# supyuxiang/Inference-Time-Scaling-for-Diffusion-Models-beyond-Scaling-Denoising-Steps

Measured on AMD Instinct MI355X. Metric: candidate-images/sec at T=1000, CIFAR-10 32x32 UNet, N=256, 1/2/4/8 MI355X, higher is better.
Workload: dtype bf16; 1 GPU; random-search round: N=256/GPU candidates x T=1000 DDPM steps, Arch A UNet 32x32 (ch128 [1,2,3,4] attn[2] nrb2), Oracle verifier; model=DDPM UNet (Diffusion/Model.py) Arch A, global_batch=256, seq_len=1000, parallelism=candidate-dp1, T=1000, graph=True, n_local=256

## Files before the change

### inference-time-scaling-for-diffusion-models-beyond-scaling-denoising-steps_amd/csrc/conv.hip

```cpp
#include <algorithm>
#include <type_traits>

#include "common.h"

namespace itsd {

constexpr int CONV_BM = 128;
constexpr int CONV_BN = 128;
constexpr int ROWB = 128;
constexpr int TILEB = 128 * ROWB;
constexpr int EROW = 132;
constexpr int EPI_BYTES = 128 * EROW * 4 + 8 * 2 * 128 * 4;
constexpr int SMEM_BYTES = (2 * 2 * TILEB > EPI_BYTES) ? 2 * 2 * TILEB : EPI_BYTES;
int g_fuse_gn = 1;
int g_conv_dbg = 0;
int g_conv_variant = 2;
int g_small_conv = 1;
int g_conv1x1 = 1;
int g_small_8x8 = 1;
int g_small_wide = 1;
int g_splitk = 1;
int g_gn_wide = 1;
int g_p4_w = 7;
int g_num_cus = 256;
// ... 1152 lines not shown
    wait_vmcnt<4>();
    __builtin_amdgcn_s_barrier();
    issue_w(s0 + 2);
    if constexpr (ST) {
      asm volatile("" ::: "memory");
      load_chunk(cc + 1);
      asm volatile("" ::: "memory");
    }
    mma_tap(s0, 0);
#pragma unroll 1
    for (int tap = 1; tap < 8; ++tap) {
      if (ST && tap <= 2) wait_vmcnt<4 + LPC>();
      else wait_vmcnt<4>();
      __builtin_amdgcn_s_barrier();
      issue_w(s0 + tap + 2);
      mma_tap(s0 + tap, tap);
    }
    wait_vmcnt<4>();
    __builtin_amdgcn_s_barrier();
    issue_w(s0 + 10);
    mma_tap(s0 + 8, 8);
    if constexpr (ST) {
      asm volatile("s_waitcnt lgkmcnt(0)" ::: "memory");
      __builtin_amdgcn_s_barrier();
      write_halo();
      asm volatile("s_waitcnt lgkmcnt(0)" ::: "memory");
    }
  };
  for (int cc = 0; cc + 1 < ncc; ++cc) run_chunk(cc, std::true_type{});
  run_chunk(ncc - 1, std::false_type{});
  wait_vmcnt<0>();
  __syncthreads();
  if (a.dbg & 16) return;
  conv_epilogue<T>(a, acc, smem, tileP, tileC);
}

#ifdef ITSD_STAMPS
__device__ unsigned long long g_stamps[1024 * 16 * 8];
__device__ __forceinline__ unsigned long long stamp() {
  __builtin_amdgcn_sched_barrier(0);
  const unsigned long long t = __builtin_amdgcn_s_memtime();
  __builtin_amdgcn_sched_barrier(0);
  return t;
}
#define STAMP(var) const unsigned long long var = stamp()
#define STAMP_ADD(slot, d) st[slot] += (d)
__device__ __forceinline__ void tl_stamp(int slot) {
  __builtin_amdgcn_sched_barrier(0);
  const unsigned long long t = (threadIdx.x >> 6) == 1 ? __builtin_amdgcn_s_memtime() : __builtin_amdgcn_s_memrealtime();
  if ((threadIdx.x & 63) == 0) g_stamps[((blockIdx.x & 1023) * 16 + (threadIdx.x >> 6)) * 8 + slot] = t;
  __builtin_amdgcn_sched_barrier(0);
}
#define TL(slot) tl_stamp(slot)
#else
#define TL(slot)
#define STAMP(var)
#define STAMP_ADD(slot, d)
#endif
constexpr int GNW_BN = 256;
constexpr int GNW_EPI = GNW_BN * EROW * 4 + (GNW_BN / 16) * 2 * CONV_BM * 4;
constexpr int GNW_SMEM = 160 * 1024;
static_assert(GNW_EPI <= GNW_SMEM, "epilogue tile");

constexpr float GN_L2E = -1.44269504f;
__device__ __forceinline__ float gn_silu_l2(float x, float a2, float b2) {
  const float t = __builtin_fmaf(x, a2, b2);
  return t * __builtin_amdgcn_rcpf(__builtin_fmaf(__builtin_amdgcn_exp2f(t), GN_L2E, GN_L2E));
}
__device__ __forceinline__ void gn_silu_x4(uint32_t xa, uint32_t xb, float a0, float a1, float a2, float a3,
                                           float b0, float b1, float b2, float b3, uint32_t zm, uint32_t& ya,
                                           uint32_t& yb) {
  float t0, t1, t2, t3, e0, e1, e2, e3;
  asm volatile(
      "v_lshlrev_b32 %2, 16, %10\n\t"
      "v_and_b32 %3, 0xffff0000, %10\n\t"
      "v_lshlrev_b32 %4, 16, %11\n\t"
      "v_and_b32 %5, 0xffff0000, %11\n\t"
      "v_fma_f32 %2, %2, %12, %16\n\t"
      "v_fma_f32 %3, %3, %13, %17\n\t"
      "v_fma_f32 %4, %4, %14, %18\n\t"
      "v_fma_f32 %5, %5, %15, %19\n\t"
      "v_exp_f32 %6, %2\n\t"
      "v_exp_f32 %7, %3\n\t"
      "v_exp_f32 %8, %4\n\t"
      "v_exp_f32 %9, %5\n\t"
      "v_fma_f32 %6, %6, %21, %21\n\t"
      "v_fma_f32 %7, %7, %21, %21\n\t"
      "v_fma_f32 %8, %8, %21, %21\n\t"
      "v_fma_f32 %9, %9, %21, %21\n\t"
      "v_rcp_f32 %6, %6\n\t"
      "v_rcp_f32 %7, %7\n\t"
      "v_rcp_f32 %8, %8\n\t"
      "v_rcp_f32 %9, %9\n\t"
      "v_mul_f32 %2, %2, %6\n\t"
      "v_mul_f32 %3, %3, %7\n\t"
      "v_mul_f32 %4, %4, %8\n\t"
      "v_mul_f32 %5, %5, %9\n\t"
      "v_cvt_pk_bf16_f32 %0, %2, %3\n\t"
      "v_cvt_pk_bf16_f32 %1, %4, %5\n\t"
      "v_and_b32 %0, %0, %20\n\t"
      "v_and_b32 %1, %1, %20"
      : "=&v"(ya), "=&v"(yb), "=&v"(t0), "=&v"(t1), "=&v"(t2), "=&v"(t3), "=&v"(e0), "=&v"(e1), "=&v"(e2),
        "=&v"(e3)
      : "v"(xa), "v"(xb), "v"(a0), "v"(a1), "v"(a2), "v"(a3), "v"(b0), "v"(b1), "v"(b2), "v"(b3), "v"(zm),
        "s"(GN_L2E));
}

template <int W> struct GnpCfg;
template <> struct GnpCfg<32> { static constexpr int NSEG = 1, ITEMS = 11, RES = 1; };
template <> struct GnpCfg<16> { static constexpr int NSEG = 1, ITEMS = 11, RES = 1; };
template <> struct GnpCfg<8> { static constexpr int NSEG = 4, ITEMS = 13, RES = 0; };


#ifndef ITSD_P4_M16
#define ITSD_P4_M16 2
#endif
#ifndef ITSD_P4_ZR8
#define ITSD_P4_ZR8 1
#endif
#ifndef ITSD_P5_SC_LAUNCH
#define ITSD_P5_SC_LAUNCH 7.5
#endif
#ifndef ITSD_P5_SWZ
#define ITSD_P5_SWZ 1
#endif
#ifndef ITSD_P4_SUBSWZ
#define ITSD_P4_SUBSWZ 1
#endif
#ifndef ITSD_P4_HSWZ
#define ITSD_P4_HSWZ 1
#endif
constexpr int P4_RING = 6;
constexpr int P4_BD = 2;
template <int W, int AB = 0>
__global__ __launch_bounds__(512, 1) void conv3x3_gn_p4_kernel(ConvArgs a) {
  typedef bf16_t T;
  constexpr bool SUB = (AB & 128) != 0, PLAIN = SUB || (AB & 2) != 0;
  constexpr bool SUB4 = SUB && (AB & 256) == 0;
  constexpr int NTAP = SUB4 ? 4 : 9, KST = 4 * NTAP;
  constexpr bool COMPACT = !SUB && (W == 8 || W == 16);
  constexpr int NSEG = GnpCfg<W>::NSEG, ITEMS = COMPACT ? 8 : GnpCfg<W>::ITEMS, RES = COMPACT ? 1 : GnpCfg<W>::RES;
  constexpr int W2 = W + 2;
  constexpr int THs = NSEG == 1 ? GNW_BN / W : W;
  constexpr int HS = (THs + 2) * W2;
  constexpr int HWs = THs * W;
  constexpr int TPS = 256 / NSEG, RPP = TPS / 8;
  constexpr int ZROW = GNW_BN;
  constexpr bool M16 = ITSD_P4_M16 >= 1 && RES && !SUB && (AB & 1) == 0 && (W == 32 || ITSD_P4_M16 >= 2);
  constexpr int ZROWS = COMPACT ? (M16 ? (ITSD_P4_ZR8 ? 72 : 65) : 1) : 0;
  auto hswz = [](int h) { return M16 && ITSD_P4_HSWZ ? (h & 6) : ((h >> 1) & 7); };
  constexpr bool CSWZ = ITSD_P4_SUBSWZ && !COMPACT && !M16 && W <= 16;
  constexpr int SC1 = 1, SC2 = W <= 8 ? 2 : 1;
  constexpr bool C96 = (AB & 512) != 0;
  constexpr int BM = C96 ? 96 : CONV_BM, HB = BM / 2, NCI = HB / 16;
  static_assert(!C96 || (M16 && COMPACT), "96-cout tiles: the 16x16x32 compact forms");
  constexpr int HALO = COMPACT ? (((GNW_BN + ZROWS) * ROWB + 1023) & ~1023) : NSEG * ITEMS * RPP * ROWB;
  constexpr int RESB = RES ? GNW_BN * CONV_BM * 2 : 0;
  static_assert(COMPACT ? ITEMS * RPP == HWs : ITEMS * RPP >= HS, "halo items cover the segment");
  constexpr int RING = ((AB & 64) || SUB) ? 4 : P4_RING, BD = (AB & 32) ? P4_BD + 1 : P4_BD;
  static_assert(KST % RING == 0, "ring slots repeat per chunk");
  __shared__ __attribute__((aligned(16))) char smem[2 * HALO + RESB + 2 * NSEG * CONV_BM * 4 + 4 * 64 * 4];
  char* const rlds = smem + 2 * HALO;
  float* const addv = (float*)(smem + 2 * HALO + RESB);
#ifdef ITSD_STAMPS
  {
    const unsigned hw = __builtin_amdgcn_s_getreg(4 | (4 << 6) | (1 << 11));
    if ((threadIdx.x & 63) == 0) g_stamps[((blockIdx.x & 1023) * 16 + 8 + (threadIdx.x >> 6)) * 8 + 1] = hw;
  }
#endif
  const int tid = threadIdx.x, lane = tid & 63;
  const int wid = __builtin_amdgcn_readfirstlane(tid >> 6);
  const int H = a.Hout;
  const int Cin = a.C1 + a.C2, ncc = Cin / 64, kpt = Cin >> 4;
  const int nTC = a.Cout / BM, nPT = a.M / GNW_BN, NT = (SUB ? 4 : 1) * nPT * nTC;
// ... 569 lines not shown
        float sm = 0.f;
#pragma unroll
        for (int i = 0; i < 2; ++i)
#pragma unroll
          for (int j = 0; j < 4; ++j)
#pragma unroll
            for (int r = 0; r < 16; ++r) sm += acc[i][j][r];
        if (sm == 1.2345f) ((float*)a.out)[0] = sm;
      }
      if constexpr (RES) {
        if (k + 1 < ntiles) init_acc(k + 1);
      } else {
#pragma unroll
        for (int i = 0; i < 2; ++i)
#pragma unroll
          for (int j = 0; j < 4; ++j)
#pragma unroll
            for (int r = 0; r < 16; ++r) acc[i][j][r] = 0.0f;
      }
      STAMP(e1);
      STAMP_ADD(6, e1 - e0);
    }
    if constexpr (RES) block_sync();
    P4_STAMP_OUT();
    return;
    }
  }

  const int tt = tid - 256, lch = tt & 7, sg = tt / TPS, lt = tt - sg * TPS;
  static_assert(COMPACT || NSEG * ITEMS * RPP > NSEG * HS, "a scratch row exists");
  if (a.dbg & (1 << 20)) __builtin_amdgcn_s_setprio(1);
  if (a.dbg & (1 << 21)) __builtin_amdgcn_s_setprio(2);
  const int dump = NSEG * HS * ROWB + (lch << 4);
  const int hrow0 = (COMPACT ? sg * HWs : sg * HS) + (lt >> 3), hrow1 = hrow0 + RPP;
  const int lds0 = hrow0 * ROWB + ((lch ^ hswz(hrow0)) << 4);
  const int lds1 = hrow1 * ROWB + ((lch ^ hswz(hrow1)) << 4);
  auto item_lds = [&](int j) {
    if constexpr (CSWZ) {
      const int r = (lt >> 3) + RPP * j, hy = r / W2, hx = r - hy * W2;
      return (sg * HS + r) * ROWB + ((lch ^ ((SC1 * hy + SC2 * hx) & 7)) << 4);
    }
    return ((j & 1) ? lds1 : lds0) + (j >> 1) * (2 * RPP * ROWB);
  };
  auto tile_y0img = [&](int k, int& img0, int& y0) {
    const int tileP = tile_p(k);
    img0 = tileP / (H * W);
    y0 = (tileP - img0 * H * W) / W;
  };
  int ipix[ITEMS];
  const float* cbase;
  int simg = 0;
  int gimg = -1;
  float* const gsw = (float*)(smem + 2 * HALO + RESB + 2 * NSEG * CONV_BM * 4) + (wid - 4) * 64;
  auto group_stats = [&](int img) __attribute__((always_inline)) {
    const int g = lane & 31, hf = Cin / 64, c0 = g * 2 * hf + (lane >> 5) * hf;
    const int HWi = H * W;
    const int sp1 = stat_spi(HWi, a.gn_spi1), sp2 = a.C2 ? stat_spi(HWi, a.gn_spi2) : 0;
    const int spm = sp1 > sp2 ? sp1 : sp2, np = hf >> 1, m = np * spm;
    double sm = 0.0, sq = 0.0;
    for (int b0 = 0; b0 < m; b0 += 8) {
      float2 vs[8], vq[8];
#pragma unroll
      for (int i = 0; i < 8; ++i) {
        const int it = b0 + i, q = it / np, cr = c0 + 2 * (it - q * np);
        const bool s1 = cr < a.C1;
        const bool ok = it < m && q < (s1 ? sp1 : sp2);
        const int c = ok ? cr : c0, qq = ok ? q : 0;
        const bool t1 = c < a.C1;
        const float* st = t1 ? a.gn_st1 : a.gn_st2;
        const int Cs = t1 ? a.C1 : a.C2, cs = t1 ? c : c - a.C1, sp = t1 ? sp1 : sp2;
        const long long slot = (long long)img * sp + qq;
        const float2 u0 = *(const float2*)(st + (slot * 2) * Cs + cs);
        const float2 u1 = *(const float2*)(st + (slot * 2 + 1) * Cs + cs);
        vs[i] = ok ? u0 : float2{0.f, 0.f};
        vq[i] = ok ? u1 : float2{0.f, 0.f};
      }
#pragma unroll
      for (int i = 0; i < 8; ++i) {
        sm += (double)vs[i].x + (double)vs[i].y;
        sq += (double)vq[i].x + (double)vq[i].y;
      }
    }
    sm += __shfl_xor(sm, 32, 64);
    sq += __shfl_xor(sq, 32, 64);
    const double E = (double)(Cin / 32) * HWi, mean = sm / E;
    double var = sq / E - mean * mean;
    var = var > 0.0 ? var : 0.0;
    if (lane < 32) {
      gsw[2 * g] = (float)mean;
      gsw[2 * g + 1] = (float)(1.0 / sqrt(var + 1e-5));
    }
  };
  auto geometry_pix = [&](int k) __attribute__((always_inline)) {
    int img0, y0;
    tile_y0img(k, img0, y0);
    int ltv = lt;
    asm volatile("" : "+v"(ltv));
#pragma unroll
    for (int j = 0; j < ITEMS; ++j) {
      const int r = (ltv >> 3) + RPP * j;
      if constexpr (COMPACT) {
        ipix[j] = (img0 + sg) * HWs + r;
      } else {
        const int hy = r / W2, hx = r - hy * W2, iy = y0 + hy - 1, ix = hx - 1;
        const bool ok = r < HS && iy >= 0 && iy < H && ix >= 0 && ix < W;
        ipix[j] = ok ? ((img0 + sg) * H + iy) * W + ix : 0;
      }
    }
    if constexpr (!PLAIN) cbase = a.gn_coef + ((size_t)(img0 + sg) * (Cin / 8) + lch) * 16;
    simg = img0 + sg;
  };
  static_assert(COMPACT || ITEMS * RPP - HS < RPP, "scratch rows only in the last item");
  const int waddr_last = (COMPACT || ((lt >> 3) + RPP * (ITEMS - 1)) < HS) ? item_lds(ITEMS - 1) : dump;
  auto waddr = [&](int j) { return j == ITEMS - 1 ? waddr_last : item_lds(j); };
  int inm = 0;
  auto geometry_emit = [&](int k) __attribute__((always_inline)) {
    int img0, y0;
    tile_y0img(k, img0, y0);
    int ltv = lt;
    asm volatile("" : "+v"(ltv));
    inm = 0;
    if constexpr (COMPACT) {
      inm = (1 << ITEMS) - 1;
      return;
    }
#pragma unroll
    for (int j = 0; j < ITEMS; ++j) {
      const int r = (ltv >> 3) + RPP * j;
      const int hy = r / W2, hx = r - hy * W2, iy = y0 + hy - 1, ix = hx - 1;
      const bool in = r >= HS || (iy >= 0 && iy < H && ix >= 0 && ix < W);
      inm |= (int)in << j;
    }
  };
  const int nrec1 = (int)std::min<long long>((long long)a.M * a.C1 * 2, 0x7fffffffLL);
  const int nrec2 = (int)std::min<long long>((long long)a.M * a.C2 * 2, 0x7fffffffLL);
  struct Src {
    __amdgpu_buffer_rsrc_t rs;
    uint32_t rowb, so;
  };
  auto src_of = [&](int cc, bool live) __attribute__((always_inline)) {
    const int ci0 = cc * 64;
    const bool s1 = ci0 < a.C1;
    Src c;
    c.rs = __builtin_amdgcn_make_buffer_rsrc(s1 ? (void*)a.src1 : (void*)a.src2, (short)0,
// ... 100 lines not shown
  };
  auto load_cn = [&](int ccx) __attribute__((always_inline)) {
    if constexpr (PLAIN) return;
    if (a.gn_fold) {
      const int c0 = ccx * 64 + 8 * lch;
      cn[0] = *(const f32x4*)(a.gn_gamma + c0);
      cn[1] = *(const f32x4*)(a.gn_gamma + c0 + 4);
      cn[2] = *(const f32x4*)(a.gn_beta + c0);
      cn[3] = *(const f32x4*)(a.gn_beta + c0 + 4);
    } else {
      const f32x4* cp = (const f32x4*)(cbase + ccx * 128);
#pragma unroll
      for (int q = 0; q < 4; ++q) cn[q] = cp[q];
    }
  };
  auto emit = [&](char* hbuf) __attribute__((always_inline)) {
    if (ccL == 0) geometry_emit(kL);
    bool opened = false;
    if (++ccL == ncc) {
      ccL = 0;
      if (++kL < ntiles) {
        geometry_pix(kL);
        opened = true;
      }
    }
    const bool live = kL < ntiles;
    load_cn(live ? ccL : 0);
    const Src nx = src_of(ccL, live);
    typedef __attribute__((ext_vector_type(2))) float f32x2;
    typedef __attribute__((ext_vector_type(2))) __bf16 bf16x2_t;
#pragma unroll
    for (int j = 0; j < ITEMS; ++j) {
      const uint32_t zm = (uint32_t)__builtin_amdgcn_sbfe(inm, j, 1);
      uint32_t yw[4];
      if constexpr (PLAIN) {
#pragma unroll
        for (int w = 0; w < 4; ++w) yw[w] = h[j][w] & zm;
      } else
#pragma unroll
      for (int hf = 0; hf < 2; ++hf)
        gn_silu_x4(h[j][2 * hf], h[j][2 * hf + 1], c[hf][0], c[hf][1], c[hf][2], c[hf][3], c[2 + hf][0],
                   c[2 + hf][1], c[2 + hf][2], c[2 + hf][3], zm, yw[2 * hf], yw[2 * hf + 1]);
      const u32x4 y = {yw[0], yw[1], yw[2], yw[3]};
      *(u32x4*)(hbuf + waddr(j)) = y;
      __builtin_amdgcn_sched_barrier(0);
      h[j] = __builtin_amdgcn_raw_buffer_load_b128(nx.rs, __umul24((uint32_t)ipix[j], nx.rowb) + lch * 16, nx.so, 0);
    }
    if (a.gn_fold && opened && simg != gimg) {
      group_stats(simg);
      gimg = simg;
    }
    prescale();
  };
  geometry_pix(0);
  {
    load_cn(0);
    const Src s0 = src_of(0, true);
#pragma unroll
    for (int j = 0; j < ITEMS; ++j)
      h[j] = __builtin_amdgcn_raw_buffer_load_b128(s0.rs, __umul24((uint32_t)ipix[j], s0.rowb) + lch * 16, s0.so, 0);
    if (a.gn_fold) group_stats(simg);
    gimg = simg;
    prescale();
  }
  if constexpr (COMPACT) {
    if (tt < 16) *(u32x4*)(smem + (tt >> 3) * HALO + ZROW * ROWB + ((tt & 7) << 4)) = u32x4{0u, 0u, 0u, 0u};
    if (M16 && ITSD_P4_ZR8) {
      const int r = (tt >> 3) & 15;
      *(u32x4*)(smem + (tt >> 7) * HALO + (ZROW + (r & 7) + (r >> 3) * 64) * ROWB + ((tt & 7) << 4)) = u32x4{0u, 0u, 0u, 0u};
    } else if (M16 && tt >= 16 && tt < 32) {
      *(u32x4*)(smem + ((tt >> 3) & 1) * HALO + (ZROW + 64) * ROWB + ((tt & 7) << 4)) = u32x4{0u, 0u, 0u, 0u};
    }
  }
  emit(smem);
#ifdef ITSD_STAMPS
  st[5] = stamp() - t_begin;
#endif
  block_sync();
  for (int q = 0, k = 0, cc = 0; q < nstages; ++q) {
    STAMP(h0);
    if (RES && cc == 1 && k > 0) {
      drain(k - 1);
      asm volatile("s_waitcnt lgkmcnt(0)" ::: "memory");
    }
    const bool res = RES && a.resid && cc == ncc - 1;
    if (res) res_dma(k);
    const int addv_cc = RES ? 0 : ncc - 1;
    if (cc == addv_cc && k + 1 < ntiles) stage_addv(k + 1, tt);
    if (q + 1 < nstages) emit(smem + ((q + 1) & 1) * HALO);
    if (res) {
      if (q + 1 < nstages) asm volatile("s_waitcnt vmcnt(%0)" ::"n"(ITEMS + 4) : "memory");
      else asm volatile("s_waitcnt vmcnt(0)" ::: "memory");
    }
#ifdef ITSD_STAMPS
    asm volatile("s_waitcnt lgkmcnt(0)" ::: "memory");
#endif
    STAMP(h1);
    STAMP_ADD(3, h1 - h0);
    block_sync();
    if (++cc == ncc) {
      cc = 0;
      ++k;
    }
  }
  if constexpr (RES) {
    block_sync();
    drain(ntiles - 1);
  }
  P4_STAMP_OUT();
}

template <int W> struct Gp5Cfg {
  static constexpr int HW = W * W;
  static constexpr bool ROWS = HW > 128;
// ... 60 lines not shown
  auto chunk_lo = [&](int z) { return z < S ? (nch * z) / S : (nchx * (z - S)) / S2; };
  auto chunk_hi = [&](int z) { return z < S ? (nch * (z + 1)) / S : (nchx * (z + 1 - S)) / S2; };
  auto block_sync = [&]() {
    asm volatile("s_waitcnt lgkmcnt(0)" ::: "memory");
    __builtin_amdgcn_s_barrier();
    asm volatile("" ::: "memory");
  };

  if (wid < 4) {
    const int rl = lane & 31, hh = lane >> 5;
    const int cw = CB == 128 ? wid : wid % CWB, jb0 = CB == 128 ? 0 : (wid / CWB) * NJW;
    int hb[NJW];
    int hq[NJW];
#pragma unroll
    for (int j = 0; j < NJW; ++j) {
      const int pl = (jb0 + j) * 32 + rl, seg = pl / SPX, rem = pl - seg * SPX, y = rem / W;
      hb[j] = seg * HS + y * W2 + (rem - y * W);
      hq[j] = SC1 * y + SC2 * (rem - y * W);
    }
    auto bunit = [&](int j, int h, int ky, int kx) {
      return W <= 16 && ITSD_P5_SWZ ? (hq[j] + SC1 * ky + SC2 * kx) & 7 : (h >> 1) & 7;
    };
    const uint32_t ablk = (uint32_t)(9 * kpt) * 1024;
    const __amdgpu_buffer_rsrc_t wrs = __builtin_amdgcn_make_buffer_rsrc((void*)a.wfrag, (short)0, 0x7fffffff, 0x00020000);
    const uint32_t avo = (uint32_t)lane * 16 + (uint32_t)cw * ablk;
    auto abase = [&](int tc, int cc) -> uint32_t { return (uint32_t)(tc * CWB) * ablk + (uint32_t)cc * 4 * 1024; };
    auto load_a = [&](uint32_t base, int st, u32x4& dst) __attribute__((always_inline)) {
#if defined(ITSD_DIAG) && defined(P5_AB)
      if constexpr ((P5_AB & 8) != 0) {
        dst = u32x4{(uint32_t)st, 0u, 0u, 0u};
        return;
      }
#endif
      dst = __builtin_amdgcn_raw_buffer_load_b128(wrs, avo, base + (uint32_t)((st >> 2) * kpt + (st & 3)) * 1024, 0);
    };
    f32x16 acc[NJW];
    u32x4 ra[P5_RING];
    const __amdgpu_buffer_rsrc_t wrx = __builtin_amdgcn_make_buffer_rsrc((void*)a.sc_wfrag, (short)0, 0x7fffffff, 0x00020000);
    const uint32_t ablkx = (uint32_t)(nchx * 4) * 1024;
    auto load_ax = [&](int tc, int cc, int st, u32x4& dst) __attribute__((always_inline)) {
      dst = __builtin_amdgcn_raw_buffer_load_b128(wrx, (uint32_t)lane * 16,
                                                  (uint32_t)(tc * CWB + cw) * ablkx + (uint32_t)(cc * 4 + st) * 1024, 0);
    };
    bool ring = false;
    {
      int tp, tc, z;
      item_of(0, tp, tc, z);
      if (z < S) {
        const uint32_t ab0 = abase(tc, chunk_lo(z));
#pragma unroll
        for (int s0 = 0; s0 < P5_RING - 1; ++s0) load_a(ab0, s0, ra[s0]);
        ring = true;
      }
    }
    block_sync();
    TL(1);
    int q = 0;
    for (int k = 0; k < nit; ++k) {
      int tp, tc, z;
      item_of(k, tp, tc, z);
      const int c0 = chunk_lo(z), c1 = chunk_hi(z);
#pragma unroll
      for (int j = 0; j < NJW; ++j)
#pragma unroll
        for (int r = 0; r < 16; ++r) acc[j][r] = 0.0f;
#if defined(ITSD_DIAG) && defined(P5_CHAINS2)
      f32x16 acc2[NJW];
#pragma unroll
      for (int j = 0; j < NJW; ++j)
#pragma unroll
        for (int r = 0; r < 16; ++r) acc2[j][r] = 0.0f;
#endif
      if (z >= S) {
#pragma unroll
        for (int st = 0; st < 4; ++st) load_ax(tc, c0, st, ra[st]);
        auto chunk1 = [&](auto pc, int cc) __attribute__((always_inline)) {
          constexpr int P = decltype(pc)::value;
          if (cc + 1 < c1) {
#pragma unroll
            for (int st = 0; st < 4; ++st) load_ax(tc, cc + 1, st, ra[4 * (1 - P) + st]);
          }
          int tx[NJW];
#pragma unroll
          for (int j = 0; j < NJW; ++j) {
            const int h = hb[j] + W2 + 1;
            tx[j] = (q & 1) * HALO + h * ROWB + ((hh ^ bunit(j, h, 1, 1)) << 4);
          }
#pragma unroll
          for (int st = 0; st < 4; ++st) {
            bf16x8 fx[NJW];
#pragma unroll
            for (int j = 0; j < NJW; ++j) fx[j] = *(const bf16x8*)(smem + (tx[j] ^ (st << 5)));
            const bf16x8 af = __builtin_bit_cast(bf16x8, ra[4 * P + st]);
#pragma unroll
            for (int j = 0; j < NJW; ++j) acc[j] = __builtin_amdgcn_mfma_f32_32x32x16_bf16(af, fx[j], acc[j], 0, 0, 0);
          }
          block_sync();
          ++q;
        };
        for (int cc = c0; cc < c1; cc += 2) {
          chunk1(std::integral_constant<int, 0>{}, cc);
          if (cc + 1 < c1) chunk1(std::integral_constant<int, 1>{}, cc + 1);
        }
        ring = false;
      } else {
      if (!ring) {
// ... 420 lines not shown
      }
      if constexpr (!DIST) TL(4);
    }
    TL(5);
    return;
  }

#if defined(ITSD_DIAG) && defined(P5_NOHALO)
  return;
#endif
  const int tt = tid - 256, lch = tt & 7, sg = tt / TPS, lt = tt - sg * TPS;
  int lds[ITEMS];
#pragma unroll
  for (int j = 0; j < ITEMS; ++j) {
    const int r = (lt >> 3) + RPP * j, hy = HY0 + r / W, x = r - (r / W) * W;
    const int hrow = sg * HS + hy * W2 + (x + 1);
    lds[j] = hrow * ROWB + ((lch ^ swz(hy, x + 1, hrow)) << 4);
  }
#ifdef ITSD_STAMPS
  {
    int m = a.M;
    asm volatile("s_waitcnt lgkmcnt(0)" : "+s"(m));
    if (m == -1) g_stamps[0] = 0;
    TL(7);
  }
#endif
  struct Src {
    __amdgpu_buffer_rsrc_t rs;
    uint32_t rowb, so;
  };
  auto src_of = [&](int cc, bool raw) __attribute__((always_inline)) {
    const int ci0 = cc * 64;
    const int C1 = raw ? static_cast<int>(a.sc_C1) : static_cast<int>(a.C1);
    const int C2 = raw ? static_cast<int>(a.sc_C2) : static_cast<int>(a.C2);
    const bool s1 = ci0 < C1;
    const void* p = raw ? (s1 ? static_cast<const void*>(a.sc_src1) : static_cast<const void*>(a.sc_src2))
                        : (s1 ? static_cast<const void*>(a.src1) : static_cast<const void*>(a.src2));
    const int nrec = (int)std::min<long long>((long long)a.M * (s1 ? C1 : C2) * 2, 0x7fffffffLL);
    Src c;
    c.rs = __builtin_amdgcn_make_buffer_rsrc((void*)p, (short)0, nrec, 0x00020000);
    c.rowb = (uint32_t)(s1 ? C1 : C2) * 2;
    c.so = (uint32_t)(s1 ? ci0 : ci0 - C1) * 2;
    return c;
  };
  u32x4 h[ITEMS];
  f32x4 c[4], cn[4];
  uint32_t zm = 0, zmn = 0;
  bool rawE = false, rawL = false;
  int kL = 0, ccL = 0, c1L = 0;
  int pix0 = 0;
  const float* cbase = a.gn_coef;
  const int hw = (tid >> 6) - 4, sw0 = (64 * hw) / TPS, sl = sg - sw0;
  float* const gsw = gsw_all + hw * 2 * SEGW * 64;
  auto group_stats = [&](int k) {
    int tp, tc, z;
    item_of(k, tp, tc, z);
    const int g = lane & 31, hf = Cin / 64, c0 = g * 2 * hf + (lane >> 5) * hf;
    const int sp1 = stat_spi(HW, a.gn_spi1), sp2 = a.C2 ? stat_spi(HW, a.gn_spi2) : 0;
    const int spm = sp1 > sp2 ? sp1 : sp2;
    static_assert(SEGW <= 2, "two segments a wave at most");
    const int np = hf >> 1, m = np * spm, mt = SEGW * m;
    int img[SEGW];
#pragma unroll
    for (int segl = 0; segl < SEGW; ++segl) {
      const int im = Cf::ROWS ? (tp * 128) / HW : tp * NSEG + sw0 + segl;
      img[segl] = im < nimg ? im : nimg - 1;
    }
    double sm0 = 0.0, sq0 = 0.0, sm1 = 0.0, sq1 = 0.0;
    for (int b0 = 0; b0 < mt; b0 += 8) {
      float2 vs[8], vq[8];
      bool hi[8];
#pragma unroll
      for (int i = 0; i < 8; ++i) {
        const int it = b0 + i;
        hi[i] = SEGW > 1 && it >= m;
        const int r = hi[i] ? it - m : it, q = r / np, cr = c0 + 2 * (r - q * np);
        const bool s1 = cr < a.C1;
        const bool ok = it < mt && q < (s1 ? sp1 : sp2);
        const int c = ok ? cr : c0, qq = ok ? q : 0;
        const bool t1 = c < a.C1;
        const float* st = t1 ? a.gn_st1 : a.gn_st2;
        const int Cs = t1 ? a.C1 : a.C2, cs = t1 ? c : c - a.C1, sp = t1 ? sp1 : sp2;
        const long long slot = (long long)(hi[i] ? img[SEGW - 1] : img[0]) * sp + qq;
        const float2 u0 = *(const float2*)(st + (slot * 2) * Cs + cs);
        const float2 u1 = *(const float2*)(st + (slot * 2 + 1) * Cs + cs);
        vs[i] = ok ? u0 : float2{0.f, 0.f};
        vq[i] = ok ? u1 : float2{0.f, 0.f};
      }
#pragma unroll
      for (int i = 0; i < 8; ++i) {
        const double ds = (double)vs[i].x + (double)vs[i].y, dq = (double)vq[i].x + (double)vq[i].y;
        if (hi[i]) {
          sm1 += ds;
          sq1 += dq;
        } else {
          sm0 += ds;
          sq0 += dq;
        }
      }
    }
#pragma unroll
    for (int segl = 0; segl < SEGW; ++segl) {
      double sm = segl ? sm1 : sm0, sq = segl ? sq1 : sq0;
      sm += __shfl_xor(sm, 32, 64);
      sq += __shfl_xor(sq, 32, 64);
      const double E = (double)(Cin / 32) * HW, mean = sm / E;
      double var = sq / E - mean * mean;
      var = var > 0.0 ? var : 0.0;
      if (lane < 32) {
        float* d = gsw + ((k & 1) * SEGW + segl) * 64 + 2 * g;
        d[0] = (float)mean;
        d[1] = (float)(1.0 / sqrt(var + 1e-5));
      }
    }
  };
  auto open_item = [&](int k) __attribute__((always_inline)) {
    int tp, tc, z;
    item_of(k, tp, tc, z);
    ccL = chunk_lo(z);
    c1L = chunk_hi(z);
    rawL = z >= S;
    const int img = Cf::ROWS ? (tp * 128) / HW : tp * NSEG + sg;
    const int y0 = Cf::ROWS ? ((tp * 128) % HW) / W : 0;
    const int imgc = img < nimg ? img : nimg - 1;
    pix0 = img * HW + (y0 - 1 + HY0) * W + (lt >> 3);
    zmn = 0;
#pragma unroll
    for (int j = 0; j < ITEMS; ++j) {
      const int y = y0 - 1 + HY0 + ((lt >> 3) + RPP * j) / W;
      zmn |= (uint32_t)(img < nimg && y >= 0 && y < W) << j;
    }
    cbase = a.gn_coef + ((size_t)imgc * (Cin / 8) + lch) * 16;
  };
  auto load_stage = [&]() __attribute__((always_inline)) {
    if (rawL) return;
    if (a.gn_fold) {
      const int c0 = ccL * 64 + 8 * lch;
      cn[0] = *(const f32x4*)(a.gn_gamma + c0);
      cn[1] = *(const f32x4*)(a.gn_gamma + c0 + 4);
      cn[2] = *(const f32x4*)(a.gn_beta + c0);
      cn[3] = *(const f32x4*)(a.gn_beta + c0 + 4);
    } else {
      const f32x4* cp = (const f32x4*)(cbase + ccL * 128);
#pragma unroll
      for (int qq = 0; qq < 4; ++qq) cn[qq] = cp[qq];
    }
  };
  auto prescale = [&]() __attribute__((always_inline)) {
    rawE = rawL;
    if (rawL) {
      zm = zmn;
      return;
    }
    if (a.gn_fold) {
      const int c0 = ccL * 64 + 8 * lch;
      const float rg = 32.0f / (float)Cin;
      const float* gs = gsw + ((kL & 1) * SEGW + sl) * 64;
#pragma unroll
      for (int e = 0; e < 8; ++e) {
        const int g = (int)(((float)(c0 + e) + 0.5f) * rg);
        const float mean = gs[2 * g], rstd = gs[2 * g + 1];
        const float sc = rstd * cn[e >> 2][e & 3];
        c[e >> 2][e & 3] = sc * GN_L2E;
        c[2 + (e >> 2)][e & 3] = (cn[2 + (e >> 2)][e & 3] - mean * sc) * GN_L2E;
      }
    } else {
#pragma unroll
// ... 18 lines not shown
    const bool live = more;
    if (live) load_stage();
    const Src nx = src_of(live ? ccL : 0, live && rawL);
#pragma unroll
    for (int j = 0; j < ITEMS; ++j) {
      uint32_t yw[4];
      const uint32_t zj = (uint32_t)__builtin_amdgcn_sbfe((int)zm, j, 1);
      if (rawE) {
#pragma unroll
        for (int e = 0; e < 4; ++e) yw[e] = h[j][e] & zj;
      } else {
#pragma unroll
        for (int hf = 0; hf < 2; ++hf)
          gn_silu_x4(h[j][2 * hf], h[j][2 * hf + 1], c[hf][0], c[hf][1], c[hf][2], c[hf][3], c[2 + hf][0],
                     c[2 + hf][1], c[2 + hf][2], c[2 + hf][3], zj, yw[2 * hf], yw[2 * hf + 1]);
      }
      *(u32x4*)(hbuf + lds[j]) = u32x4{yw[0], yw[1], yw[2], yw[3]};
      __builtin_amdgcn_sched_barrier(0);
      const uint32_t pix = live && ((zmn >> j) & 1) ? (uint32_t)(pix0 + RPP * j) : 0u;
      h[j] = __builtin_amdgcn_raw_buffer_load_b128(nx.rs, __umul24(pix, nx.rowb) + lch * 16, nx.so, 0);
    }
    prescale();
    if (live) advance();
  };
  auto stage_addv = [&](int k) {
    int tp, tc, z;
    item_of(k, tp, tc, z);
    const long long trow = a.temb ? (a.temb_tsel ? (long long)(*a.temb_tsel) * a.temb_row_stride : 0) : 0;
    for (int it = tt; it < NSEG * CB; it += 256) {
      const int il = it / CB, cl = it % CB, co = tc * CB + cl;
      const int img = min(Cf::ROWS ? (tp * 128) / HW : tp * NSEG + il, nimg - 1);
      float v = a.bias[co];
      if (a.temb) v += a.temb[trow + (long long)img * a.temb_img_stride + co];
      if (a.cemb) {
        int lab = 0;
        if (a.cemb_uncond_from < 0 || img < a.cemb_uncond_from) lab = a.cemb_labels[img % a.cemb_label_mod];
        v += a.cemb[(long long)lab * a.cemb_row_stride + co];
      }
      addv[(k & 1) * NSEG * CONV_BM + it] = v;
    }
  };
  auto res_dma = [&](int k) __attribute__((always_inline)) {
    int tp, tc, z;
    item_of(k, tp, tc, z);
    const int hw = (tid >> 6) - 4;
#pragma unroll
    for (int i = 0; i < 8; ++i) {
      const int r0 = 4 * (8 * hw + i), r = r0 + (lane >> 4), u = (lane & 15) ^ (r & 15), p = tp * 128 + r;
      const T* src = p < a.M && u * 8 < CB ? (const T*)a.resid + (size_t)p * a.Cout + tc * CB + u * 8
                                           : (const T*)zero_of_block<T>(a);
      __builtin_amdgcn_global_load_lds((const void*)src, (lds_ptr_t)(rres + (k & 1) * RTILE + r0 * 256), 16, 0, 0);
    }
  };
  open_item(0);
  load_stage();
  {
    const Src s0 = src_of(ccL, rawL);
#pragma unroll
    for (int j = 0; j < ITEMS; ++j)
      h[j] = __builtin_amdgcn_raw_buffer_load_b128(
          s0.rs, __umul24(((zmn >> j) & 1) ? (uint32_t)(pix0 + RPP * j) : 0u, s0.rowb) + lch * 16, s0.so, 0);
  }
  for (int u = tt; u < 2 * NSEG * HS * 8; u += 256) {
    const int row = (u >> 3) % (NSEG * HS), buf = (u >> 3) / (NSEG * HS), r = row % HS, y = r / W2, x = r - y * W2;
    if (x == 0 || x == W2 - 1 || (!Cf::ROWS && (y == 0 || y == TH + 1)))
      *(u32x4*)(smem + buf * HALO + row * ROWB + ((u & 7) << 4)) = u32x4{0u, 0u, 0u, 0u};
  }
  if (a.gn_fold && !rawL) group_stats(0);
  TL(1);
  prescale();
  advance();
  emit(smem);
  TL(2);
  block_sync();
  TL(3);
  int q = 0;
  for (int k = 0; k < nit; ++k) {
    int tp, tc, z;
    item_of(k, tp, tc, z);
    const int c0 = chunk_lo(z), c1 = chunk_hi(z);
    for (int cc = c0; cc < c1; ++cc, ++q) {
      if (cc == c0) stage_addv(k);
      const bool rdma = a.resid && cc + 1 == c1;
      if (rdma) res_dma(k);
      const bool em = !(k + 1 == nit && cc + 1 == c1);
      if (em) emit(smem + ((q + 1) & 1) * HALO);
      if (rdma) {
        if (em) asm volatile("s_waitcnt vmcnt(%0)" ::"n"(ITEMS) : "memory");
        else asm volatile("s_waitcnt vmcnt(0)" ::: "memory");
      }
      if (q == 0) TL(4);
      block_sync();
      if (q == 0) TL(6);
    }
  }
  TL(5);
}

__global__ __launch_bounds__(256) void gn_coef_kernel(GNArgs g, float* coef) {
  __shared__ float gst[32][2];
  const int img = blockIdx.x, tid = threadIdx.x;
  const int C = g.C1 + g.C2, gsz = C / 32;
  const int spi1 = stat_spi(g.HW, g.spi1), spi2 = stat_spi(g.HW, g.spi2);
  float gam[8], bet[8];
#pragma unroll
  for (int u = 0; u < 8; ++u) {
    const int c = tid + 256 * u;
    gam[u] = c < C ? g.gamma[c] : 0.f;
    bet[u] = c < C ? g.beta[c] : 0.f;
  }
  {
    const int grp = tid >> 3, l8 = tid & 7;
    const int c0 = grp * gsz, nc1 = max(0, min(g.C1 - c0, gsz)), n1 = nc1 * spi1, n = n1 + (gsz - nc1) * spi2;
    double s = 0.0, q = 0.0;
    for (int k = l8; k < n; k += 8) {
      const bool s1 = k < n1;
      const int spi = s1 ? spi1 : spi2, kk = s1 ? k : k - n1;
      const int c = c0 + (s1 ? 0 : nc1) + kk / spi;
      const long long sl = (long long)img * spi + (kk % spi);
      const float* st = s1 ? g.st1 : g.st2;
      const int Cs = s1 ? g.C1 : g.C2, cs = s1 ? c : c - g.C1;
// ... 564 lines not shown
```

Before: 61.93 candidate-images/sec.

## Prefetch GroupNorm statistics early in fused conv prologue and move halo zeroing

```diff
diff --git a/inference-time-scaling-for-diffusion-models-beyond-scaling-denoising-steps_amd/csrc/conv.hip b/inference-time-scaling-for-diffusion-models-beyond-scaling-denoising-steps_amd/csrc/conv.hip
--- a/inference-time-scaling-for-diffusion-models-beyond-scaling-denoising-steps_amd/csrc/conv.hip
+++ b/inference-time-scaling-for-diffusion-models-beyond-scaling-denoising-steps_amd/csrc/conv.hip
@@ -1228,8 +1228,10 @@
   __builtin_amdgcn_sched_barrier(0);
 }
 #define TL(slot) tl_stamp(slot)
+#define TLX(slot) tl_stamp(64 + (slot))
 #else
 #define TL(slot)
+#define TLX(slot)
 #define STAMP(var)
 #define STAMP_ADD(slot, d)
 #endif
@@ -1296,6 +1298,9 @@
 #endif
 #ifndef ITSD_P5_SC_LAUNCH
 #define ITSD_P5_SC_LAUNCH 7.5
+#endif
+#ifndef ITSD_STAT_CAP
+#define ITSD_STAT_CAP 32
 #endif
 #ifndef ITSD_P5_SWZ
 #define ITSD_P5_SWZ 1
@@ -1971,44 +1976,118 @@
   int simg = 0;
   int gimg = -1;
   float* const gsw = (float*)(smem + 2 * HALO + RESB + 2 * NSEG * CONV_BM * 4) + (wid - 4) * 64;
-  auto group_stats = [&](int img) __attribute__((always_inline)) {
-    const int g = lane & 31, hf = Cin / 64, c0 = g * 2 * hf + (lane >> 5) * hf;
-    const int HWi = H * W;
-    const int sp1 = stat_spi(HWi, a.gn_spi1), sp2 = a.C2 ? stat_spi(HWi, a.gn_spi2) : 0;
-    const int spm = sp1 > sp2 ? sp1 : sp2, np = hf >> 1, m = np * spm;
-    double sm = 0.0, sq = 0.0;
-    for (int b0 = 0; b0 < m; b0 += 8) {
-      float2 vs[8], vq[8];
-#pragma unroll
-      for (int i = 0; i < 8; ++i) {
-        const int it = b0 + i, q = it / np, cr = c0 + 2 * (it - q * np);
-        const bool s1 = cr < a.C1;
-        const bool ok = it < m && q < (s1 ? sp1 : sp2);
-        const int c = ok ? cr : c0, qq = ok ? q : 0;
-        const bool t1 = c < a.C1;
-        const float* st = t1 ? a.gn_st1 : a.gn_st2;
-        const int Cs = t1 ? a.C1 : a.C2, cs = t1 ? c : c - a.C1, sp = t1 ? sp1 : sp2;
-        const long long slot = (long long)img * sp + qq;
-        const float2 u0 = *(const float2*)(st + (slot * 2) * Cs + cs);
-        const float2 u1 = *(const float2*)(st + (slot * 2 + 1) * Cs + cs);
-        vs[i] = ok ? u0 : float2{0.f, 0.f};
-        vq[i] = ok ? u1 : float2{0.f, 0.f};
-      }
-#pragma unroll
-      for (int i = 0; i < 8; ++i) {
-        sm += (double)vs[i].x + (double)vs[i].y;
-        sq += (double)vq[i].x + (double)vq[i].y;
-      }
-    }
+  struct StatGeo {
+    int c0, sp1, sp2, np, m;
+  };
+  auto stats_geo = [&]() __attribute__((always_inline)) {
+    StatGeo s;
+    const int hf = Cin / 64, HWi = H * W;
+    s.c0 = (lane & 31) * 2 * hf + (lane >> 5) * hf;
+    s.sp1 = stat_spi(HWi, a.gn_spi1);
+    s.sp2 = a.C2 ? stat_spi(HWi, a.gn_spi2) : 0;
+    s.np = hf >> 1;
+    s.m = s.np * (s.sp1 > s.sp2 ? s.sp1 : s.sp2);
+    return s;
+  };
+  auto stats_load = [&](const StatGeo& s, int img, int q, int p, bool in, float2& u0, float2& u1) __attribute__((always_inline)) {
+    const int cr = s.c0 + 2 * p;
+    const bool s1 = cr < a.C1;
+    const bool ok = in && q < (s1 ? s.sp1 : s.sp2);
+    const int c = ok ? cr : s.c0, qq = ok ? q : 0;
+    const bool t1 = c < a.C1;
+    const float* st = t1 ? a.gn_st1 : a.gn_st2;
+    const int Cs = t1 ? a.C1 : a.C2, cs = t1 ? c : c - a.C1, sp = t1 ? s.sp1 : s.sp2;
+    const long long slot = (long long)img * sp + qq;
+    u0 = *(const float2*)(st + (slot * 2) * Cs + cs);
+    u1 = *(const float2*)(st + (slot * 2 + 1) * Cs + cs);
+    return ok;
+  };
+  auto stats_add = [&](bool ok, float2 u0, float2 u1, double& sm, double& sq) __attribute__((always_inline)) {
+    const float2 vs = ok ? u0 : float2{0.f, 0.f}, vq = ok ? u1 : float2{0.f, 0.f};
+    sm += (double)vs.x + (double)vs.y;
+    sq += (double)vq.x + (double)vq.y;
+  };
+  auto stats_write = [&](double sm, double sq) __attribute__((always_inline)) {
     sm += __shfl_xor(sm, 32, 64);
     sq += __shfl_xor(sq, 32, 64);
-    const double E = (double)(Cin / 32) * HWi, mean = sm / E;
+    const double E = (double)(Cin / 32) * (H * W), mean = sm / E;
     double var = sq / E - mean * mean;
     var = var > 0.0 ? var : 0.0;
     if (lane < 32) {
-      gsw[2 * g] = (float)mean;
-      gsw[2 * g + 1] = (float)(1.0 / sqrt(var + 1e-5));
-    }
+      gsw[2 * (lane & 31)] = (float)mean;
+      gsw[2 * (lane & 31) + 1] = (float)(1.0 / sqrt(var + 1e-5));
+    }
+  };
+  auto group_stats = [&](int img) __attribute__((always_inline)) {
+    const StatGeo s = stats_geo();
+    double sm = 0.0, sq = 0.0;
+    for (int b0 = 0; b0 < s.m; b0 += 8) {
+      float2 u0[8], u1[8];
+      bool ok[8];
+#pragma unroll
+      for (int i = 0; i < 8; ++i) {
+        const int it = b0 + i, q = it / s.np;
+        ok[i] = stats_load(s, img, q, it - q * s.np, it < s.m, u0[i], u1[i]);
+      }
+#pragma unroll
+      for (int i = 0; i < 8; ++i) stats_add(ok[i], u0[i], u1[i], sm, sq);
+    }
+    stats_write(sm, sq);
+  };
+  constexpr int P4_SCAP = ITSD_STAT_CAP;
+  auto stats_issue = [&](const StatGeo& s, int img, int g0, float2 (&su0)[P4_SCAP], float2 (&su1)[P4_SCAP]) __attribute__((always_inline)) {
+    uint32_t sok = 0;
+    int q = g0 / s.np, p = g0 - q * s.np;
+    const float* const b1 = a.gn_st1 + ((long long)img * s.sp1 * 2) * a.C1;
+    const float* const b2 = a.gn_st2 + ((long long)img * s.sp2 * 2) * a.C2;
+    auto load = [&](int q, int p, bool in, float2& u0, float2& u1) __attribute__((always_inline)) {
+      const int cr = s.c0 + 2 * p;
+      const bool s1 = cr < a.C1;
+      const bool ok = in && q < (s1 ? s.sp1 : s.sp2);
+      const int c = ok ? cr : s.c0, qq = ok ? q : 0;
+      const bool t1 = c < a.C1;
+      const float* st = t1 ? b1 : b2;
+      const int Cs = t1 ? a.C1 : a.C2, off = qq * 2 * Cs + (t1 ? c : c - a.C1);
+      u0 = *(const float2*)(st + off);
+      u1 = *(const float2*)(st + off + Cs);
+      return ok;
+    };
+#pragma unroll
+    for (int bb = 0; bb < P4_SCAP; bb += 8) {
+      if (g0 + bb < s.m) {
+#pragma unroll
+        for (int i = 0; i < 8; ++i) {
+          sok |= (uint32_t)load(q, p, g0 + bb + i < s.m, su0[bb + i], su1[bb + i]) << (bb + i);
+          __builtin_amdgcn_sched_barrier(0);
+          if (++p == s.np) {
+            p = 0;
+            ++q;
+          }
+        }
+      }
+    }
+    return sok;
+  };
+  auto stats_sum = [&](const StatGeo& s, int g0, uint32_t sok, const float2 (&su0)[P4_SCAP], const float2 (&su1)[P4_SCAP],
+                       double& sm, double& sq) __attribute__((always_inline)) {
+#pragma unroll
+    for (int bb = 0; bb < P4_SCAP; bb += 8) {
+      if (g0 + bb < s.m) {
+#pragma unroll
+        for (int i = 0; i < 8; ++i) stats_add((sok >> (bb + i)) & 1, su0[bb + i], su1[bb + i], sm, sq);
+      }
+    }
+  };
+  auto stats_finish = [&](const StatGeo& s, int img, uint32_t sok, const float2 (&su0)[P4_SCAP], const float2 (&su1)[P4_SCAP])
+                          __attribute__((always_inline)) {
+    double sm = 0.0, sq = 0.0;
+    stats_sum(s, 0, sok, su0, su1, sm, sq);
+    for (int g0 = P4_SCAP; g0 < s.m; g0 += P4_SCAP) {
+      float2 t0[P4_SCAP], t1[P4_SCAP];
+      const uint32_t tok = stats_issue(s, img, g0, t0, t1);
+      stats_sum(s, g0, tok, t0, t1, sm, sq);
+    }
+    stats_write(sm, sq);
   };
   auto geometry_pix = [&](int k) __attribute__((always_inline)) {
     int img0, y0;
@@ -2215,6 +2294,15 @@
     }
     prescale();
   };
+  StatGeo geo0{};
+  float2 su0[P4_SCAP], su1[P4_SCAP];
+  uint32_t sok = 0;
+  if (a.gn_fold) {
+    int img0, y0;
+    tile_y0img(0, img0, y0);
+    geo0 = stats_geo();
+    sok = stats_issue(geo0, img0 + sg, 0, su0, su1);
+  }
   geometry_pix(0);
   {
     load_cn(0);
@@ -2222,7 +2310,7 @@
 #pragma unroll
     for (int j = 0; j < ITEMS; ++j)
       h[j] = __builtin_amdgcn_raw_buffer_load_b128(s0.rs, __umul24((uint32_t)ipix[j], s0.rowb) + lch * 16, s0.so, 0);
-    if (a.gn_fold) group_stats(simg);
+    if (a.gn_fold) stats_finish(geo0, simg, sok, su0, su1);
     gimg = simg;
     prescale();
   }
@@ -2389,6 +2477,11 @@
         for (int s0 = 0; s0 < P5_RING - 1; ++s0) load_a(ab0, s0, ra[s0]);
         ring = true;
       }
+    }
+    for (int u = tid; u < 2 * NSEG * HS * 8; u += 256) {
+      const int row = (u >> 3) % (NSEG * HS), buf = (u >> 3) / (NSEG * HS), r = row % HS, y = r / W2, x = r - y * W2;
+      if (x == 0 || x == W2 - 1 || (!Cf::ROWS && (y == 0 || y == TH + 1)))
+        *(u32x4*)(smem + buf * HALO + row * ROWB + ((u & 7) << 4)) = u32x4{0u, 0u, 0u, 0u};
     }
     block_sync();
     TL(1);
@@ -2915,67 +3008,152 @@
   const float* cbase = a.gn_coef;
   const int hw = (tid >> 6) - 4, sw0 = (64 * hw) / TPS, sl = sg - sw0;
   float* const gsw = gsw_all + hw * 2 * SEGW * 64;
-  auto group_stats = [&](int k) {
+  static_assert(SEGW <= 2, "two segments a wave at most");
+  struct StatGeo {
+    int c0, sp1, sp2, np, m, mt;
+    int img[SEGW];
+  };
+  auto stats_geo = [&](int k) __attribute__((always_inline)) {
     int tp, tc, z;
     item_of(k, tp, tc, z);
-    const int g = lane & 31, hf = Cin / 64, c0 = g * 2 * hf + (lane >> 5) * hf;
-    const int sp1 = stat_spi(HW, a.gn_spi1), sp2 = a.C2 ? stat_spi(HW, a.gn_spi2) : 0;
-    const int spm = sp1 > sp2 ? sp1 : sp2;
-    static_assert(SEGW <= 2, "two segments a wave at most");
-    const int np = hf >> 1, m = np * spm, mt = SEGW * m;
-    int img[SEGW];
+    StatGeo s;
+    const int hf = Cin / 64;
+    s.c0 = (lane & 31) * 2 * hf + (lane >> 5) * hf;
+    s.sp1 = stat_spi(HW, a.gn_spi1);
+    s.sp2 = a.C2 ? stat_spi(HW, a.gn_spi2) : 0;
+    s.np = hf >> 1;
+    s.m = s.np * (s.sp1 > s.sp2 ? s.sp1 : s.sp2);
+    s.mt = SEGW * s.m;
 #pragma unroll
     for (int segl = 0; segl < SEGW; ++segl) {
       const int im = Cf::ROWS ? (tp * 128) / HW : tp * NSEG + sw0 + segl;
-      img[segl] = im < nimg ? im : nimg - 1;
-    }
-    double sm0 = 0.0, sq0 = 0.0, sm1 = 0.0, sq1 = 0.0;
-    for (int b0 = 0; b0 < mt; b0 += 8) {
-      float2 vs[8], vq[8];
-      bool hi[8];
-#pragma unroll
-      for (int i = 0; i < 8; ++i) {
-        const int it = b0 + i;
-        hi[i] = SEGW > 1 && it >= m;
-        const int r = hi[i] ? it - m : it, q = r / np, cr = c0 + 2 * (r - q * np);
-        const bool s1 = cr < a.C1;
-        const bool ok = it < mt && q < (s1 ? sp1 : sp2);
-        const int c = ok ? cr : c0, qq = ok ? q : 0;
-        const bool t1 = c < a.C1;
-        const float* st = t1 ? a.gn_st1 : a.gn_st2;
-        const int Cs = t1 ? a.C1 : a.C2, cs = t1 ? c : c - a.C1, sp = t1 ? sp1 : sp2;
-        const long long slot = (long long)(hi[i] ? img[SEGW - 1] : img[0]) * sp + qq;
-        const float2 u0 = *(const float2*)(st + (slot * 2) * Cs + cs);
-        const float2 u1 = *(const float2*)(st + (slot * 2 + 1) * Cs + cs);
-        vs[i] = ok ? u0 : float2{0.f, 0.f};
-        vq[i] = ok ? u1 : float2{0.f, 0.f};
-      }
-#pragma unroll
-      for (int i = 0; i < 8; ++i) {
-        const double ds = (double)vs[i].x + (double)vs[i].y, dq = (double)vq[i].x + (double)vq[i].y;
-        if (hi[i]) {
-          sm1 += ds;
-          sq1 += dq;
-        } else {
-          sm0 += ds;
-          sq0 += dq;
-        }
-      }
-    }
+      s.img[segl] = im < nimg ? im : nimg - 1;
+    }
+    return s;
+  };
+  auto stats_load = [&](const StatGeo& s, bool hi, int q, int p, bool in, float2& u0, float2& u1) __attribute__((always_inline)) {
+    const int cr = s.c0 + 2 * p;
+    const bool s1 = cr < a.C1;
+    const bool ok = in && q < (s1 ? s.sp1 : s.sp2);
+    const int c = ok ? cr : s.c0, qq = ok ? q : 0;
+    const bool t1 = c < a.C1;
+    const float* st = t1 ? a.gn_st1 : a.gn_st2;
+    const int Cs = t1 ? a.C1 : a.C2, cs = t1 ? c : c - a.C1, sp = t1 ? s.sp1 : s.sp2;
+    const long long slot = (long long)(hi ? s.img[SEGW - 1] : s.img[0]) * sp + qq;
+    u0 = *(const float2*)(st + (slot * 2) * Cs + cs);
+    u1 = *(const float2*)(st + (slot * 2 + 1) * Cs + cs);
+    return ok;
+  };
+  auto stats_add = [&](bool hi, bool ok, float2 u0, float2 u1, double (&sm)[2], double (&sq)[2]) __attribute__((always_inline)) {
+    const float2 vs = ok ? u0 : float2{0.f, 0.f}, vq = ok ? u1 : float2{0.f, 0.f};
+    const double ds = (double)vs.x + (double)vs.y, dq = (double)vq.x + (double)vq.y;
+    if (hi) {
+      sm[1] += ds;
+      sq[1] += dq;
+    } else {
+      sm[0] += ds;
+      sq[0] += dq;
+    }
+  };
+  auto stats_write = [&](int k, const double (&sm2)[2], const double (&sq2)[2]) __attribute__((always_inline)) {
 #pragma unroll
     for (int segl = 0; segl < SEGW; ++segl) {
-      double sm = segl ? sm1 : sm0, sq = segl ? sq1 : sq0;
+      double sm = sm2[segl], sq = sq2[segl];
       sm += __shfl_xor(sm, 32, 64);
       sq += __shfl_xor(sq, 32, 64);
       const double E = (double)(Cin / 32) * HW, mean = sm / E;
       double var = sq / E - mean * mean;
       var = var > 0.0 ? var : 0.0;
       if (lane < 32) {
-        float* d = gsw + ((k & 1) * SEGW + segl) * 64 + 2 * g;
+        float* d = gsw + ((k & 1) * SEGW + segl) * 64 + 2 * (lane & 31);
         d[0] = (float)mean;
         d[1] = (float)(1.0 / sqrt(var + 1e-5));
       }
     }
+  };
+  auto group_stats = [&](int k) {
+    const StatGeo s = stats_geo(k);
+    double sm[2] = {0.0, 0.0}, sq[2] = {0.0, 0.0};
+    for (int b0 = 0; b0 < s.mt; b0 += 8) {
+      float2 u0[8], u1[8];
+      bool hi[8], ok[8];
+#pragma unroll
+      for (int i = 0; i < 8; ++i) {
+        const int it = b0 + i;
+        hi[i] = SEGW > 1 && it >= s.m;
+        const int r = hi[i] ? it - s.m : it, q = r / s.np;
+        ok[i] = stats_load(s, hi[i], q, r - q * s.np, it < s.mt, u0[i], u1[i]);
+      }
+#pragma unroll
+      for (int i = 0; i < 8; ++i) stats_add(hi[i], ok[i], u0[i], u1[i], sm, sq);
+    }
+    stats_write(k, sm, sq);
+  };
+  constexpr int P5_SCAP = W == 16 && DIST && ITSD_STAT_CAP > 24 ? 24 : ITSD_STAT_CAP;
+  auto stats_issue = [&](const StatGeo& s, int g0, float2 (&su0)[P5_SCAP], float2 (&su1)[P5_SCAP]) __attribute__((always_inline)) {
+    uint32_t sok = 0;
+    bool hi = SEGW > 1 && g0 >= s.m;
+    int q = (hi ? g0 - s.m : g0) / s.np, p = (hi ? g0 - s.m : g0) - q * s.np;
+    const int im0 = hi ? s.img[SEGW - 1] : s.img[0];
+    const float* b1 = a.gn_st1 + ((long long)im0 * s.sp1 * 2) * a.C1;
+    const float* b2 = a.gn_st2 + ((long long)im0 * s.sp2 * 2) * a.C2;
+    auto load = [&](bool hi, int q, int p, bool in, float2& u0, float2& u1) __attribute__((always_inline)) {
+      const int cr = s.c0 + 2 * p;
+      const bool s1 = cr < a.C1;
+      const bool ok = in && q < (s1 ? s.sp1 : s.sp2);
+      const int c = ok ? cr : s.c0, qq = ok ? q : 0;
+      const bool t1 = c < a.C1;
+      const float* st = t1 ? b1 : b2;
+      const int Cs = t1 ? a.C1 : a.C2, off = qq * 2 * Cs + (t1 ? c : c - a.C1);
+      u0 = *(const float2*)(st + off);
+      u1 = *(const float2*)(st + off + Cs);
+      return ok;
+    };
+#pragma unroll
+    for (int bb = 0; bb < P5_SCAP; bb += 8) {
+      if (g0 + bb < s.mt) {
+#pragma unroll
+        for (int i = 0; i < 8; ++i) {
+          const int it = g0 + bb + i;
+          sok |= (uint32_t)load(hi, q, p, it < s.mt, su0[bb + i], su1[bb + i]) << (bb + i);
+          __builtin_amdgcn_sched_barrier(0);
+          if (++p == s.np) {
+            p = 0;
+            ++q;
+          }
+          if (SEGW > 1 && it + 1 == s.m) {
+            hi = true;
+            q = 0;
+            p = 0;
+            b1 = a.gn_st1 + ((long long)s.img[SEGW - 1] * s.sp1 * 2) * a.C1;
+            b2 = a.gn_st2 + ((long long)s.img[SEGW - 1] * s.sp2 * 2) * a.C2;
+          }
+        }
+      }
+    }
+    return sok;
+  };
+  auto stats_sum = [&](const StatGeo& s, int g0, uint32_t sok, const float2 (&su0)[P5_SCAP], const float2 (&su1)[P5_SCAP],
+                       double (&sm)[2], double (&sq)[2]) __attribute__((always_inline)) {
+#pragma unroll
+    for (int bb = 0; bb < P5_SCAP; bb += 8) {
+      if (g0 + bb < s.mt) {
+#pragma unroll
+        for (int i = 0; i < 8; ++i)
+          stats_add(SEGW > 1 && g0 + bb + i >= s.m, (sok >> (bb + i)) & 1, su0[bb + i], su1[bb + i], sm, sq);
+      }
+    }
+  };
+  auto stats_finish = [&](const StatGeo& s, int k, uint32_t sok, const float2 (&su0)[P5_SCAP], const float2 (&su1)[P5_SCAP])
+                          __attribute__((always_inline)) {
+    double sm[2] = {0.0, 0.0}, sq[2] = {0.0, 0.0};
+    stats_sum(s, 0, sok, su0, su1, sm, sq);
+    for (int g0 = P5_SCAP; g0 < s.mt; g0 += P5_SCAP) {
+      float2 t0[P5_SCAP], t1[P5_SCAP];
+      const uint32_t tok = stats_issue(s, g0, t0, t1);
+      stats_sum(s, g0, tok, t0, t1, sm, sq);
+    }
+    stats_write(k, sm, sq);
   };
   auto open_item = [&](int k) __attribute__((always_inline)) {
     int tp, tc, z;
@@ -3100,6 +3278,19 @@
       __builtin_amdgcn_global_load_lds((const void*)src, (lds_ptr_t)(rres + (k & 1) * RTILE + r0 * 256), 16, 0, 0);
     }
   };
+  StatGeo geo0{};
+  float2 su0[P5_SCAP], su1[P5_SCAP];
+  uint32_t sok = 0;
+  bool st0 = false;
+  if (a.gn_fold) {
+    int tp, tc, z;
+    item_of(0, tp, tc, z);
+    st0 = z < S;
+  }
+  if (st0) {
+    geo0 = stats_geo(0);
+    sok = stats_issue(geo0, 0, su0, su1);
+  }
   open_item(0);
   load_stage();
   {
@@ -3109,12 +3300,8 @@
       h[j] = __builtin_amdgcn_raw_buffer_load_b128(
           s0.rs, __umul24(((zmn >> j) & 1) ? (uint32_t)(pix0 + RPP * j) : 0u, s0.rowb) + lch * 16, s0.so, 0);
   }
-  for (int u = tt; u < 2 * NSEG * HS * 8; u += 256) {
-    const int row = (u >> 3) % (NSEG * HS), buf = (u >> 3) / (NSEG * HS), r = row % HS, y = r / W2, x = r - y * W2;
-    if (x == 0 || x == W2 - 1 || (!Cf::ROWS && (y == 0 || y == TH + 1)))
-      *(u32x4*)(smem + buf * HALO + row * ROWB + ((u & 7) << 4)) = u32x4{0u, 0u, 0u, 0u};
-  }
-  if (a.gn_fold && !rawL) group_stats(0);
+  TLX(2);
+  if (st0) stats_finish(geo0, 0, sok, su0, su1);
   TL(1);
   prescale();
   advance();
```

After: 62.48 candidate-images/sec, median of 6. Within noise of the previous version (+0.9%).
